# Future-Power-Networks/MAPDN

Hardware: AMD Instinct MI355X
Metric: env-steps/sec (whole node), case141 batch=4096, at 1/2/4/8 MI355X (higher is better)
Workload: dtype f64

## Files before the change

### mapdn_amd/csrc/critic.hip

```cpp
#include <hip/hip_runtime.h>
#include <stdint.h>

#include <algorithm>
#include <cstdlib>

#include "../../include/mapdn.h"
#include "rowtile.hpp"

namespace mapdn {

template <bool BC>
__device__ __forceinline__ void load_row(const HeadArgs& p, long row, int g, f4 (&xa)[4]) {
  if (BC) {
    const unsigned q = (unsigned)row / (unsigned)p.n, i = (unsigned)row - q * (unsigned)p.n;
    const float* pb = p.x + (size_t)q * 64 + 4 * g;
    const float* pn = p.per_n + (size_t)i * 64 + 4 * g;
#pragma unroll
    for (int c = 0; c < 4; ++c) xa[c] = *(const f4*)(pb + 16 * c) + *(const f4*)(pn + 16 * c);
  } else {
    const float* px = p.x + (size_t)row * 64 + 4 * g;
#pragma unroll
    for (int c = 0; c < 4; ++c) xa[c] = *(const f4*)(px + 16 * c);
  }
}

template <bool BC>
__global__ void __launch_bounds__(256)
k_head_fwd(HeadArgs p, float* __restrict__ v, long rows) {
  const int lane = threadIdx.x & 63, wave = threadIdx.x >> 6, g = lane >> 4, j = lane & 15;
  f4 wop[4][4], gam[4], bet[4], b2v[4], w3v[4];
#pragma unroll
  for (int nt = 0; nt < 4; ++nt) {
#pragma unroll
    for (int c = 0; c < 4; ++c) wop[nt][c] = *(const f4*)(p.w2 + (size_t)(16 * nt + j) * 64 + 16 * c + 4 * g);
    gam[nt] = *(const f4*)(p.gamma + 16 * nt + 4 * g); bet[nt] = *(const f4*)(p.beta + 16 * nt + 4 * g);
    b2v[nt] = *(const f4*)(p.b2 + 16 * nt + 4 * g); w3v[nt] = *(const f4*)(p.w3 + 16 * nt + 4 * g);
  }
  const float b3 = p.b3[0];
  const long n_tiles = (rows + 15) >> 4;
  for (long T = (long)blockIdx.x * 4 + wave; T < n_tiles; T += (long)gridDim.x * 4) {
    const long row = T * 16 + j;
    f4 xa[4];
    load_row<BC>(p, row < rows ? row : rows - 1, g, xa);
    ln_stats(xa, p.eps);
#pragma unroll
    for (int c = 0; c < 4; ++c) {
      const f4 y = xa[c] * gam[c] + bet[c];
      xa[c] = f4{relu_nan(y.x), relu_nan(y.y), relu_nan(y.z), relu_nan(y.w)};
    }
    f4 acc[4] = {f4{0, 0, 0, 0}, f4{0, 0, 0, 0}, f4{0, 0, 0, 0}, f4{0, 0, 0, 0}};
#pragma unroll
    for (int c = 0; c < 4; ++c)
#pragma unroll
      for (int q = 0; q < 4; ++q)
#pragma unroll
        for (int nt = 0; nt < 4; ++nt) acc[nt] = __builtin_amdgcn_mfma_f32_16x16x4f32(wop[nt][c][q], xa[c][q], acc[nt], 0, 0, 0);
    float dot = 0.0f;
#pragma unroll
    for (int nt = 0; nt < 4; ++nt)
#pragma unroll
      for (int r = 0; r < 4; ++r) dot = fmaf(relu_nan(acc[nt][r] + b2v[nt][r]), w3v[nt][r], dot);
    dot = sum_g(dot);
    if (g == 0 && row < rows) v[row] = dot + b3;
  }
}

template <bool BC, int MODE, int NT>
__global__ void __launch_bounds__(NT)
k_head_bwd(HeadArgs p, const float* __restrict__ dv, float* __restrict__ dx, const float* __restrict__ dot_w, float* __restrict__ dact,
           float* __restrict__ partial, int pstride, long rows, const float* __restrict__ wrow, const float* __restrict__ scale) {
  constexpr bool PG = MODE == 0 || MODE == 3;
  constexpr int NW = NT / 64, TILES = NT == 512 ? 1 : 2;
  constexpr bool SLIM = NT == 512;
  extern __shared__ float sm[];
  f4* sW = (f4*)sm;
  f4* sWT = sW + 1024;
  float* sP = (float*)(sWT + 1024);
  float* stage = sP + 256 + (size_t)(threadIdx.x >> 6) * TILES * 16 * HS;
  float* accn = sP + 256 + (size_t)NW * TILES * 16 * HS + (size_t)(threadIdx.x >> 6) * p.n * 64;
  const int tid = threadIdx.x, lane = tid & 63, wave = tid >> 6, g = lane >> 4, j = lane & 15;
  if (tid < 64) { sP[tid] = p.gamma[tid]; sP[64 + tid] = p.beta[tid]; sP[128 + tid] = p.b2[tid]; sP[192 + tid] = p.w3[tid]; }
  for (int i = tid; i < 1024; i += NT) {
    const int l = i & 63, c = (i >> 6) & 3, nt = i >> 8, lj = l & 15, lg = l >> 4;
    sW[i] = *(const f4*)(p.w2 + (size_t)(16 * nt + lj) * 64 + 16 * c + 4 * lg);
    f4 t;
#pragma unroll
    for (int q = 0; q < 4; ++q) t[q] = p.w2[(size_t)(16 * c + 4 * lg + q) * 64 + 16 * nt + lj];
    sWT[i] = t;
  }
  if (BC && MODE != 2) for (int i = lane; i < p.n * 64; i += 64) accn[i] = 0.0f;
  f4 gam_[4], bet_[4], b2v_[4], w3v_[4];
#pragma unroll
  for (int nt = 0; nt < 4; ++nt) {
    gam_[nt] = *(const f4*)(p.gamma + 16 * nt + 4 * g); bet_[nt] = *(const f4*)(p.beta + 16 * nt + 4 * g);
    b2v_[nt] = *(const f4*)(p.b2 + 16 * nt + 4 * g); w3v_[nt] = *(const f4*)(p.w3 + 16 * nt + 4 * g);
  }
  __syncthreads();
  auto GAM = [&](int c) -> f4 { return SLIM ? *(const f4*)(sP + 16 * c + 4 * g) : gam_[c]; };
  auto BET = [&](int c) -> f4 { return SLIM ? *(const f4*)(sP + 64 + 16 * c + 4 * g) : bet_[c]; };
  auto B2V = [&](int c) -> f4 { return SLIM ? *(const f4*)(sP + 128 + 16 * c + 4 * g) : b2v_[c]; };
  auto W3V = [&](int c) -> f4 { return SLIM ? *(const f4*)(sP + 192 + 16 * c + 4 * g) : w3v_[c]; };

  const long W = (long)gridDim.x * NW, w = (long)blockIdx.x * NW + wave;
  long r0, r1;
  if (BC) { const long G = rows / p.n; r0 = (G * w / W) * p.n; r1 = (G * (w + 1) / W) * p.n; }
  else { const long Tn = (rows + 15) >> 4; r0 = (Tn * w / W) * 16; r1 = (Tn * (w + 1) / W) * 16; if (r1 > rows) r1 = rows; }

  f4 accW[4][4];
  f4 ag[4], ab[4], aw3[4], ab2[4];
  float ab3 = 0.0f, carry = 0.0f;
  float aloss = 0.0f;
  const float b3 = MODE == 3 ? p.b3[0] : 0.0f, lscale = MODE == 3 ? scale[0] : 0.0f;
#pragma unroll
  for (int a = 0; a < 4; ++a) {
#pragma unroll
    for (int b = 0; b < 4; ++b) accW[a][b] = f4{0, 0, 0, 0};
    ag[a] = ab[a] = aw3[a] = ab2[a] = f4{0, 0, 0, 0};
  }

  f4 xnext[4];
  float dvnext = 0.0f;
  if (!SLIM && r0 < r1) {
    const long row = r0 + j;
    load_row<BC>(p, row < r1 ? row : r1 - 1, g, xnext);
    dvnext = row < r1 ? dv[row] : 0.0f;
  }
  for (long row0 = r0; row0 < r1; row0 += 16) {
    const long row = row0 + j;
    const bool valid = row < r1;
    f4 xh[4];
    float dvcur;
    if (SLIM) {
      load_row<BC>(p, valid ? row : r1 - 1, g, xh);
      dvcur = valid ? dv[row] : 0.0f;
    } else {
#pragma unroll
      for (int c = 0; c < 4; ++c) xh[c] = xnext[c];
      dvcur = dvnext;
      if (row0 + 16 < r1) {
        const long rn = row + 16;
        load_row<BC>(p, rn < r1 ? rn : r1 - 1, g, xnext);
        dvnext = rn < r1 ? dv[rn] : 0.0f;
      }
    }
    const float rs = ln_stats(xh, p.eps);
    f4 xn[4];
#pragma unroll
    for (int c = 0; c < 4; ++c) {
      const f4 y = xh[c] * GAM(c) + BET(c);
      xn[c] = f4{relu_nan(y.x), relu_nan(y.y), relu_nan(y.z), relu_nan(y.w)};
    }
    f4 acc[4] = {f4{0, 0, 0, 0}, f4{0, 0, 0, 0}, f4{0, 0, 0, 0}, f4{0, 0, 0, 0}};
#pragma unroll
    for (int c = 0; c < 4; ++c) {
      f4 wv[4];
#pragma unroll
      for (int nt = 0; nt < 4; ++nt) wv[nt] = sW[(nt * 4 + c) * 64 + lane];
#pragma unroll
      for (int q = 0; q < 4; ++q)
#pragma unroll
        for (int nt = 0; nt < 4; ++nt) acc[nt] = __builtin_amdgcn_mfma_f32_16x16x4f32(wv[nt][q], xn[c][q], acc[nt], 0, 0, 0);
    }
    float dvr = dvcur;
    if (MODE == 3) {
      float dot = 0.0f;
#pragma unroll
      for (int nt = 0; nt < 4; ++nt) {
        const f4 bb = B2V(nt), ww = W3V(nt);
#pragma unroll
        for (int r = 0; r < 4; ++r) dot = fmaf(relu_nan(acc[nt][r] + bb[r]), ww[r], dot);
      }
      const float err = dvcur - (sum_g(dot) + b3);
      float wgt = lscale;
      if (wrow) { const unsigned rc = (unsigned)(valid ? row : r1 - 1); wgt *= wrow[BC ? rc / (unsigned)p.n : rc]; }
      dvr = valid ? -2.0f * wgt * err : 0.0f;
      if (valid && g == 0) aloss = fmaf(wgt * err, err, aloss);
    }
#pragma unroll
    for (int nt = 0; nt < 4; ++nt) {
      const f4 bb = B2V(nt), ww = W3V(nt);
#pragma unroll
      for (int r = 0; r < 4; ++r) {
        const float pre = acc[nt][r] + bb[r];
        const bool pos = pre > 0.0f;
        const float dp = pos ? dvr * ww[r] : 0.0f;
        if (PG) { aw3[nt][r] = fmaf(pos ? pre : 0.0f, dvr, aw3[nt][r]); ab2[nt][r] += dp; }
        acc[nt][r] = dp;
      }
    }
    if (PG && g == 0) ab3 += dvr;
    f4 dxn[4] = {f4{0, 0, 0, 0}, f4{0, 0, 0, 0}, f4{0, 0, 0, 0}, f4{0, 0, 0, 0}};
#pragma unroll
    for (int c = 0; c < 4; ++c) {
      f4 wv[4];
#pragma unroll
      for (int nt = 0; nt < 4; ++nt) wv[nt] = sWT[(nt * 4 + c) * 64 + lane];
#pragma unroll
      for (int q = 0; q < 4; ++q)
#pragma unroll
        for (int nt = 0; nt < 4; ++nt) dxn[nt] = __builtin_amdgcn_mfma_f32_16x16x4f32(wv[nt][q], acc[c][q], dxn[nt], 0, 0, 0);
    }
    if (PG) {
      float* s0 = stage; float* s1 = SLIM ? stage : stage + 16 * HS;
#pragma unroll
      for (int c = 0; c < 4; ++c) *(f4*)(s0 + j * HS + 16 * c + 4 * g) = acc[c];
      if (!SLIM) {
#pragma unroll
        for (int c = 0; c < 4; ++c) *(f4*)(s1 + j * HS + 16 * c + 4 * g) = xn[c];
      }
      __builtin_amdgcn_fence(__ATOMIC_RELEASE, "wavefront");
      __builtin_amdgcn_wave_barrier();
      __builtin_amdgcn_fence(__ATOMIC_ACQUIRE, "wavefront");
      float dCs[4][4];
      if (SLIM) {
#pragma unroll
        for (int s = 0; s < 4; ++s)
#pragma unroll
          for (int nt = 0; nt < 4; ++nt) dCs[s][nt] = s0[(4 * g + s) * HS + 16 * nt + j];
        __builtin_amdgcn_fence(__ATOMIC_RELEASE, "wavefront");
        __builtin_amdgcn_wave_barrier();
#pragma unroll
        for (int c = 0; c < 4; ++c) *(f4*)(s1 + j * HS + 16 * c + 4 * g) = xn[c];
        __builtin_amdgcn_fence(__ATOMIC_RELEASE, "wavefront");
        __builtin_amdgcn_wave_barrier();
        __builtin_amdgcn_fence(__ATOMIC_ACQUIRE, "wavefront");
      }
#pragma unroll
      for (int s = 0; s < 4; ++s) {
        float dC[4], xC[4];
#pragma unroll
        for (int nt = 0; nt < 4; ++nt) { dC[nt] = SLIM ? dCs[s][nt] : s0[(4 * g + s) * HS + 16 * nt + j]; xC[nt] = s1[(4 * g + s) * HS + 16 * nt + j]; }
#pragma unroll
        for (int a = 0; a < 4; ++a)
#pragma unroll
          for (int b = 0; b < 4; ++b) accW[a][b] = __builtin_amdgcn_mfma_f32_16x16x4f32(dC[a], xC[b], accW[a][b], 0, 0, 0);
      }
    }
    float s1a = 0.0f, s2a = 0.0f;
#pragma unroll
    for (int c = 0; c < 4; ++c) {
      f4 d;
#pragma unroll
      for (int q = 0; q < 4; ++q) d[q] = xn[c][q] > 0.0f ? dxn[c][q] : 0.0f;
      if (PG) { ag[c] += d * xh[c]; ab[c] += d; }
      const f4 a = d * GAM(c);
      s1a += hsum(a); s2a += hsum(a * xh[c]);
      dxn[c] = a;
    }
    const float m1 = sum_g(s1a) * (1.0f / 64.0f), m2 = sum_g(s2a) * (1.0f / 64.0f);
#pragma unroll
    for (int c = 0; c < 4; ++c) dxn[c] = (dxn[c] - m1 - xh[c] * m2) * rs;
    if (MODE == 2) {
      const unsigned i = BC ? (unsigned)((valid ? row : r1 - 1) - r0) % (unsigned)p.n : 0u;
      const float* pw = dot_w + (size_t)i * 64 + 4 * g;
      float d = 0.0f;
#pragma unroll
      for (int c = 0; c < 4; ++c) d += hsum(dxn[c] * *(const f4*)(pw + 16 * c));
      d = sum_g(d);
      if (g == 0 && valid) dact[row] = d;
    } else if (!BC) {
      if (valid) {
        float* px = dx + (size_t)row * 64 + 4 * g;
#pragma unroll
        for (int c = 0; c < 4; ++c) *(f4*)(px + 16 * c) = dxn[c];
      }
    } else {
      float* s0 = stage;
      __builtin_amdgcn_fence(__ATOMIC_RELEASE, "wavefront");
      __builtin_amdgcn_wave_barrier();
#pragma unroll
      for (int c = 0; c < 4; ++c) *(f4*)(s0 + j * HS + 16 * c + 4 * g) = dxn[c];
      __builtin_amdgcn_fence(__ATOMIC_RELEASE, "wavefront");
      __builtin_amdgcn_wave_barrier();
      __builtin_amdgcn_fence(__ATOMIC_ACQUIRE, "wavefront");
      const int cnt = (int)(r1 - row0 < 16 ? r1 - row0 : 16);
      const unsigned rel = (unsigned)(row0 - r0);
      unsigned grp = rel / (unsigned)p.n, i = rel - grp * (unsigned)p.n;
      float* pbase = dx + ((size_t)(r0 / p.n) + grp) * 64 + lane;
      if (p.n >= 16) {
        unsigned i2 = i;
        constexpr int H = SLIM ? 4 : 16;
#pragma unroll
        for (int h0 = 0; h0 < 16; h0 += H) {
          float val[H], cur[H];
#pragma unroll
          for (int rr = 0; rr < H; ++rr) {
            unsigned ii = i + h0 + rr; if (ii >= (unsigned)p.n) ii -= p.n;
            val[rr] = h0 + rr < cnt ? s0[(h0 + rr) * HS + lane] : 0.0f;
            cur[rr] = accn[ii * 64 + lane];
          }
#pragma unroll
          for (int rr = 0; rr < H; ++rr) {
            unsigned ii = i + h0 + rr; if (ii >= (unsigned)p.n) ii -= p.n;
            accn[ii * 64 + lane] = cur[rr] + val[rr];
          }
#pragma unroll
          for (int rr = 0; rr < H; ++rr)
            if (h0 + rr < cnt) {
              carry += val[rr];
              if (++i2 == (unsigned)p.n) { *pbase = carry; carry = 0.0f; i2 = 0; pbase += 64; }
            }
        }
      } else {
        for (int rr = 0; rr < cnt; ++rr) {
          const float val = s0[rr * HS + lane];
          carry += val;
          accn[i * 64 + lane] += val;
          if (++i == (unsigned)p.n) { *pbase = carry; carry = 0.0f; i = 0; pbase += 64; }
        }
      }
      __builtin_amdgcn_fence(__ATOMIC_RELEASE, "wavefront");
      __builtin_amdgcn_wave_barrier();
    }
  }

  if (MODE != 2) {
    float* pp = partial + (size_t)blockIdx.x * pstride;
    if (BC) {
      __syncthreads();
      const float* a0 = sP + 256 + (size_t)NW * TILES * 16 * HS;
      for (int i = tid; i < p.n * 64; i += NT) {
        float t = a0[i];
#pragma unroll
        for (int ww = 1; ww < NW; ++ww) t += a0[(size_t)ww * p.n * 64 + i];
        pp[HP + i] = t;
      }
    }
    if (PG) {
      __syncthreads();
      float* red = sm + (size_t)wave * HP;
#pragma unroll
      for (int a = 0; a < 4; ++a)
#pragma unroll
        for (int b = 0; b < 4; ++b)
#pragma unroll
          for (int r = 0; r < 4; ++r) red[(16 * a + 4 * g + r) * 64 + 16 * b + j] = accW[a][b][r];
#pragma unroll
      for (int c = 0; c < 4; ++c)
#pragma unroll
        for (int q = 0; q < 4; ++q) {
          const float tg = sum_j(ag[c][q]), tb = sum_j(ab[c][q]), t2 = sum_j(ab2[c][q]), t3 = sum_j(aw3[c][q]);
          if (j == 0) {
            const int col = 16 * c + 4 * g + q;
            red[4096 + col] = tg; red[4160 + col] = tb; red[4224 + col] = t2; red[4288 + col] = t3;
          }
        }
      const float t = sum_j(ab3), tl = sum_j(aloss);
      if (lane == 0) { red[4352] = t; red[4353] = tl; }
      __syncthreads();
      for (int col = tid; col < HW; col += NT) {
        float v = sm[col];
#pragma unroll
        for (int ww = 1; ww < NW; ++ww) v += sm[(size_t)ww * HP + col];
        pp[col] = v;
      }
    }
  }
}

__global__ void __launch_bounds__(256) k_head_reduce(const float* __restrict__ partial, int nw, int pstride, int lo, int hi, int written,
                                                     float* __restrict__ out) {
  __shared__ float s_acc[4][64];
  const int c = threadIdx.x & 63, grp = threadIdx.x >> 6, col = lo + blockIdx.x * 64 + c;
  float acc = 0.0f;
  if (col < written) for (int i = grp; i < nw; i += 4) acc += partial[(size_t)i * pstride + col];
  s_acc[grp][c] = acc;
  __syncthreads();
  if (grp == 0 && col < hi) out[col] = (s_acc[0][c] + s_acc[1][c]) + (s_acc[2][c] + s_acc[3][c]);
}

}

static int head_cus() {
  int dev = 0, cus = 256;
  if (hipGetDevice(&dev) == hipSuccess) (void)hipDeviceGetAttribute(&cus, hipDeviceAttributeMultiprocessorCount, dev);
  return cus;
}
static int head_bwd_blocks(int64_t rows, int32_t n, bool bc, int nw, int cus = 0) {
  const int64_t units = bc ? rows / n : (rows + 15) / 16;
  return (int)std::max<int64_t>(1, std::min<int64_t>((units + nw - 1) / nw, cus ? cus : head_cus()));
}
static size_t head_bwd_lds(int threads, int32_t n, bool accn) {
  const int nw = threads / 64, tiles = threads == 512 ? 1 : 2;
  return (size_t)2 * 1024 * 16 + 256 * 4 + (size_t)nw * tiles * 16 * mapdn::HS * 4 + (accn ? (size_t)nw * n * 64 * 4 : 0);
}
static int head_bwd_threads(int64_t rows, int32_t n, bool bc, bool accn, int cus = 0) {
  const char* e = getenv("MAPDN_HEAD_BWD_THREADS");
  const bool fits = head_bwd_lds(512, n, accn) <= (size_t)160 * 1024;
  if (e && atoi(e) == 256) return 256;
  if (e && atoi(e) == 512 && fits) return 512;
  const int64_t units = bc ? rows / n : (rows + 15) / 16;
  return fits && units >= (int64_t)(cus ? cus : head_cus()) * 8 ? 512 : 256;
}
static bool head_args_ok(const float* x, const float* per_n, int32_t n, const float* gamma, const float* beta, const float* w2, const float* b2,
                         const float* w3, const float* b3, int64_t rows) {
  if (!x || !gamma || !beta || !w2 || !b2 || !w3 || !b3 || rows < 1 || rows > 0x7fffffff) return false;
  if (per_n && (n < 1 || n > 256 || rows % n)) return false;
  return true;
}

extern "C" int mapdn_critic_head_forward(const float* x, const float* per_n, int32_t n, const float* gamma, const float* beta, float eps,
                                         const float* w2, const float* b2, const float* w3, const float* b3, float* v, int64_t rows,
                                         void* stream) {
  using namespace mapdn;
  if (!head_args_ok(x, per_n, n, gamma, beta, w2, b2, w3, b3, rows) || !v) return MAPDN_E_INVALID;
  const HeadArgs a{x, per_n, per_n ? n : 1, gamma, beta, eps, w2, b2, w3, b3};
  const int64_t tiles = (rows + 15) / 16;
  const int blocks = (int)std::max<int64_t>(1, std::min<int64_t>((tiles + 3) / 4, (int64_t)head_cus() * 2));
  if (per_n) hipLaunchKernelGGL(k_head_fwd<true>, dim3(blocks), dim3(256), 0, (hipStream_t)stream, a, v, (long)rows);
  else hipLaunchKernelGGL(k_head_fwd<false>, dim3(blocks), dim3(256), 0, (hipStream_t)stream, a, v, (long)rows);
  return hipGetLastError() == hipSuccess ? MAPDN_OK : MAPDN_E_HIP;
}

extern "C" int64_t mapdn_critic_head_scratch_floats(int64_t rows, int32_t n, int32_t formed) {
  if (rows < 1 || (formed && (n < 1 || rows % n))) return 0;
  const int64_t blocks = std::max<int64_t>(head_bwd_blocks(rows, n, formed != 0, 4), head_bwd_blocks(rows, n, formed != 0, 8));
  return blocks * (mapdn::HP + (formed ? n * 64 : 0));
}

extern "C" int mapdn_critic_head_backward_geometry(int64_t rows, int32_t n, int32_t formed, int32_t mode, int32_t cus, int32_t* threads,
                                                   int32_t* blocks, int32_t* lds_bytes) {
  if (rows < 1 || rows > 0x7fffffff || mode < 0 || mode > 3 || cus < 0 || (formed && (n < 1 || n > 256 || rows % n))) return MAPDN_E_INVALID;
  const bool bc = formed != 0;
  if (!bc) n = 1;
  const int c = cus ? cus : head_cus();
  const int nt = head_bwd_threads(rows, n, bc, bc && mode != 2, c);
  size_t lds = head_bwd_lds(nt, n, bc && mode != 2);
  if (mode == 0 || mode == 3) lds = std::max(lds, (size_t)(nt / 64) * mapdn::HP * 4);
  if (lds > (size_t)160 * 1024) return MAPDN_E_INVALID;
  if (threads) *threads = nt;
  if (blocks) *blocks = head_bwd_blocks(rows, n, bc, nt / 64, c);
  if (lds_bytes) *lds_bytes = (int32_t)lds;
  return MAPDN_OK;
}

template <bool BC, int MODE, int NT>
static int head_bwd_launch_nt(const mapdn::HeadArgs& a, const float* dv, float* dx, const float* dot_w, float* dact, float* scratch, float* grads,
                              int64_t rows, hipStream_t st, const float* wrow, const float* scale) {
  using namespace mapdn;
  constexpr int NW = NT / 64;
  const int blocks = head_bwd_blocks(rows, a.n, BC, NW), nw = blocks;
  const int pstride = HP + (BC ? a.n * 64 : 0);
  size_t lds = head_bwd_lds(NT, a.n, BC && MODE != 2);
  if (MODE == 0 || MODE == 3) lds = std::max(lds, (size_t)NW * HP * 4);
  if (lds > (size_t)160 * 1024) return MAPDN_E_INVALID;
  const void* fn = (const void*)k_head_bwd<BC, MODE, NT>;
  if (hipFuncSetAttribute(fn, hipFuncAttributeMaxDynamicSharedMemorySize, 160 * 1024) != hipSuccess) return MAPDN_E_HIP;
  hipLaunchKernelGGL((k_head_bwd<BC, MODE, NT>), dim3(blocks), dim3(NT), lds, st, a, dv, dx, dot_w, dact, scratch, pstride, (long)rows, wrow, scale);
  if (MODE == 0 || MODE == 3) hipLaunchKernelGGL(k_head_reduce, dim3((HP + 63) / 64), dim3(256), 0, st, scratch, nw, pstride, 0, HP, HW, grads);
  if (BC && MODE != 2) hipLaunchKernelGGL(k_head_reduce, dim3(a.n), dim3(256), 0, st, scratch, nw, pstride, HP, HP + a.n * 64, HP + a.n * 64, grads);
  return hipGetLastError() == hipSuccess ? MAPDN_OK : MAPDN_E_HIP;
}
template <bool BC, int MODE>
static int head_bwd_launch(const mapdn::HeadArgs& a, const float* dv, float* dx, const float* dot_w, float* dact, float* scratch, float* grads,
                           int64_t rows, hipStream_t st, const float* wrow = nullptr, const float* scale = nullptr) {
  if (head_bwd_threads(rows, a.n, BC, BC && MODE != 2) == 512)
    return head_bwd_launch_nt<BC, MODE, 512>(a, dv, dx, dot_w, dact, scratch, grads, rows, st, wrow, scale);
  return head_bwd_launch_nt<BC, MODE, 256>(a, dv, dx, dot_w, dact, scratch, grads, rows, st, wrow, scale);
}

extern "C" int mapdn_critic_head_backward(const float* dv, const float* x, const float* per_n, int32_t n, const float* gamma, const float* beta,
                                          float eps, const float* w2, const float* b2, const float* w3, const float* b3, float* dx, float* grads,
                                          float* scratch, int64_t rows, int32_t param_grads, void* stream) {
  using namespace mapdn;
  if (!head_args_ok(x, per_n, n, gamma, beta, w2, b2, w3, b3, rows) || !dv || !dx || ((param_grads || per_n) && (!grads || !scratch)))
    return MAPDN_E_INVALID;
  const HeadArgs a{x, per_n, per_n ? n : 1, gamma, beta, eps, w2, b2, w3, b3};
  hipStream_t st = (hipStream_t)stream;
  if (per_n) return param_grads ? head_bwd_launch<true, 0>(a, dv, dx, nullptr, nullptr, scratch, grads, rows, st)
                                : head_bwd_launch<true, 1>(a, dv, dx, nullptr, nullptr, scratch, grads, rows, st);
  return param_grads ? head_bwd_launch<false, 0>(a, dv, dx, nullptr, nullptr, scratch, grads, rows, st)
                     : head_bwd_launch<false, 1>(a, dv, dx, nullptr, nullptr, scratch, grads, rows, st);
}

extern "C" int mapdn_critic_head_backward_dot(const float* dv, const float* x, const float* per_n, int32_t n, const float* gamma,
                                              const float* beta, float eps, const float* w2, const float* b2, const float* w3, const float* b3,
                                              const float* dot_w, float* dact, int64_t rows, void* stream) {
  using namespace mapdn;
  if (!head_args_ok(x, per_n, n, gamma, beta, w2, b2, w3, b3, rows) || !dv || !dot_w || !dact) return MAPDN_E_INVALID;
  const HeadArgs a{x, per_n, per_n ? n : 1, gamma, beta, eps, w2, b2, w3, b3};
  hipStream_t st = (hipStream_t)stream;
  return per_n ? head_bwd_launch<true, 2>(a, dv, nullptr, dot_w, dact, nullptr, nullptr, rows, st)
               : head_bwd_launch<false, 2>(a, dv, nullptr, dot_w, dact, nullptr, nullptr, rows, st);
}

extern "C" int mapdn_critic_head_mse(const float* ret, const float* wrow, const float* scale, const float* x, const float* per_n, int32_t n,
                                     const float* gamma, const float* beta, float eps, const float* w2, const float* b2, const float* w3,
                                     const float* b3, float* dx, float* grads, float* scratch, int64_t rows, void* stream) {
  using namespace mapdn;
  if (!head_args_ok(x, per_n, n, gamma, beta, w2, b2, w3, b3, rows) || !ret || !scale || !dx || !grads || !scratch) return MAPDN_E_INVALID;
  const HeadArgs a{x, per_n, per_n ? n : 1, gamma, beta, eps, w2, b2, w3, b3};
  hipStream_t st = (hipStream_t)stream;
  return per_n ? head_bwd_launch<true, 3>(a, ret, dx, nullptr, nullptr, scratch, grads, rows, st, wrow, scale)
               : head_bwd_launch<false, 3>(a, ret, dx, nullptr, nullptr, scratch, grads, rows, st, wrow, scale);
}

#include "critic_twin.hip"
#include "critic_cf.hip"
#include "critic_attn.hip"
```

Baseline: 39.98 million.

## Restructure critic backward row fetch with incremental indexing and vectorized staging

Replaces per-row integer division and modulo for broadcast group indexing with incrementally advanced counters, and folds row-weight and per-n loads into a unified prefetch lambda. LDS staging of activations and gradients now uses f4 vector reads with a transposed layout, and the xn store is moved earlier to overlap with the MFMA work. The weight-gradient reduction layout changes to match the new layout. It also swaps the relu helper and uses readfirstlane for the wave index. These changes aim to cut scalar address arithmetic and scalar LDS traffic, at the risk of subtle indexing or layout mismatches.

```diff
diff --git a/mapdn_amd/csrc/critic.hip b/mapdn_amd/csrc/critic.hip
--- a/mapdn_amd/csrc/critic.hip
+++ b/mapdn_amd/csrc/critic.hip
@@ -23,6 +23,18 @@
     for (int c = 0; c < 4; ++c) xa[c] = *(const f4*)(px + 16 * c);
   }
 }
+
+__device__ __forceinline__ float relu_keep(float o) { return !(o <= 0.0f) ? o : 0.0f; }
+
+__device__ __forceinline__ f4 ln_affine(f4 xh, f4 gam, f4 bet) {
+  return f4{fmaf(xh.x, gam.x, bet.x), fmaf(xh.y, gam.y, bet.y), fmaf(xh.z, gam.z, bet.z), fmaf(xh.w, gam.w, bet.w)};
+}
+
+__device__ __forceinline__ void stage_put(float* t, int j, int g, const f4 (&v)[4]) {
+#pragma unroll
+  for (int c = 0; c < 4; ++c) *(f4*)(t + j * HS + 16 * c + 4 * g) = v[c];
+}
+__device__ __forceinline__ f4 stage_get(const float* t, int j, int g, int s) { return *(const f4*)(t + (4 * g + s) * HS + 4 * j); }
 
 template <bool BC>
 __global__ void __launch_bounds__(256)
@@ -46,7 +58,7 @@
 #pragma unroll
     for (int c = 0; c < 4; ++c) {
       const f4 y = xa[c] * gam[c] + bet[c];
-      xa[c] = f4{relu_nan(y.x), relu_nan(y.y), relu_nan(y.z), relu_nan(y.w)};
+      xa[c] = f4{relu_keep(y.x), relu_keep(y.y), relu_keep(y.z), relu_keep(y.w)};
     }
     f4 acc[4] = {f4{0, 0, 0, 0}, f4{0, 0, 0, 0}, f4{0, 0, 0, 0}, f4{0, 0, 0, 0}};
 #pragma unroll
@@ -59,7 +71,7 @@
 #pragma unroll
     for (int nt = 0; nt < 4; ++nt)
 #pragma unroll
-      for (int r = 0; r < 4; ++r) dot = fmaf(relu_nan(acc[nt][r] + b2v[nt][r]), w3v[nt][r], dot);
+      for (int r = 0; r < 4; ++r) dot = fmaf(relu_keep(acc[nt][r] + b2v[nt][r]), w3v[nt][r], dot);
     dot = sum_g(dot);
     if (g == 0 && row < rows) v[row] = dot + b3;
   }
@@ -76,9 +88,9 @@
   f4* sW = (f4*)sm;
   f4* sWT = sW + 1024;
   float* sP = (float*)(sWT + 1024);
-  float* stage = sP + 256 + (size_t)(threadIdx.x >> 6) * TILES * 16 * HS;
-  float* accn = sP + 256 + (size_t)NW * TILES * 16 * HS + (size_t)(threadIdx.x >> 6) * p.n * 64;
-  const int tid = threadIdx.x, lane = tid & 63, wave = tid >> 6, g = lane >> 4, j = lane & 15;
+  const int tid = threadIdx.x, lane = tid & 63, wave = __builtin_amdgcn_readfirstlane(tid >> 6), g = lane >> 4, j = lane & 15;
+  float* stage = sP + 256 + (size_t)wave * TILES * 16 * HS;
+  float* accn = sP + 256 + (size_t)NW * TILES * 16 * HS + (size_t)wave * p.n * 64;
   if (tid < 64) { sP[tid] = p.gamma[tid]; sP[64 + tid] = p.beta[tid]; sP[128 + tid] = p.b2[tid]; sP[192 + tid] = p.w3[tid]; }
   for (int i = tid; i < 1024; i += NT) {
     const int l = i & 63, c = (i >> 6) & 3, nt = i >> 8, lj = l & 15, lg = l >> 4;
@@ -118,37 +130,61 @@
     ag[a] = ab[a] = aw3[a] = ab2[a] = f4{0, 0, 0, 0};
   }
 
-  f4 xnext[4];
-  float dvnext = 0.0f;
-  if (!SLIM && r0 < r1) {
-    const long row = r0 + j;
-    load_row<BC>(p, row < r1 ? row : r1 - 1, g, xnext);
-    dvnext = row < r1 ? dv[row] : 0.0f;
-  }
+  const unsigned un = (unsigned)p.n, dq = 16u / un, di = 16u % un;
+  const unsigned g0 = BC ? (unsigned)(r0 / p.n) : 0u, qlast = BC ? (unsigned)((r1 - 1) / p.n) : 0u;
+  unsigned fq = BC ? g0 + (unsigned)j / un : 0u, fi = BC ? (unsigned)j % un : 0u, fg = g0, fti = 0, tg = g0, ti = 0;
+
+  f4 nxa[4], nxb[4];
+  float ndv = 0.0f, nwr = 1.0f;
+  unsigned ni = 0;
+  auto fetch = [&](long row0f) {
+    const bool ok = row0f + j < r1;
+    const char* xb;
+    unsigned rel;
+    if (BC) {
+      rel = (ok ? fq : qlast) - fg;
+      ni = ok ? fi : un - 1;
+      xb = (const char*)(p.x + (size_t)fg * 64);
+      const unsigned poff = ni * 256u + 16u * g;
+#pragma unroll
+      for (int c = 0; c < 4; ++c) nxb[c] = *(const f4*)((const char*)p.per_n + poff + 64 * c);
+      if (MODE == 3 && wrow) nwr = *(const float*)((const char*)(wrow + fg) + 4u * rel);
+      fi += di; fq += dq;
+      if (fi >= un) { fi -= un; ++fq; }
+      fti += di; fg += dq;
+      if (fti >= un) { fti -= un; ++fg; }
+    } else {
+      rel = ok ? (unsigned)j : (unsigned)(r1 - 1 - row0f);
+      xb = (const char*)(p.x + (size_t)row0f * 64);
+      if (MODE == 3 && wrow) nwr = *(const float*)((const char*)(wrow + row0f) + 4u * rel);
+    }
+    const unsigned off = rel * 256u + 16u * g;
+#pragma unroll
+    for (int c = 0; c < 4; ++c) nxa[c] = *(const f4*)(xb + off + 64 * c);
+    ndv = ok ? *(const float*)((const char*)(dv + row0f) + 4u * j) : 0.0f;
+  };
+  if (!SLIM && r0 < r1) fetch(r0);
   for (long row0 = r0; row0 < r1; row0 += 16) {
-    const long row = row0 + j;
-    const bool valid = row < r1;
+    const bool valid = row0 + j < r1;
+    if (SLIM) fetch(row0);
     f4 xh[4];
-    float dvcur;
-    if (SLIM) {
-      load_row<BC>(p, valid ? row : r1 - 1, g, xh);
-      dvcur = valid ? dv[row] : 0.0f;
-    } else {
-#pragma unroll
-      for (int c = 0; c < 4; ++c) xh[c] = xnext[c];
-      dvcur = dvnext;
-      if (row0 + 16 < r1) {
-        const long rn = row + 16;
-        load_row<BC>(p, rn < r1 ? rn : r1 - 1, g, xnext);
-        dvnext = rn < r1 ? dv[rn] : 0.0f;
-      }
-    }
+#pragma unroll
+    for (int c = 0; c < 4; ++c) xh[c] = BC ? nxa[c] + nxb[c] : nxa[c];
+    const float dvcur = ndv, wcur = nwr;
+    const unsigned icur = ni;
+    if (!SLIM && row0 + 16 < r1) fetch(row0 + 16);
     const float rs = ln_stats(xh, p.eps);
     f4 xn[4];
 #pragma unroll
     for (int c = 0; c < 4; ++c) {
-      const f4 y = xh[c] * GAM(c) + BET(c);
-      xn[c] = f4{relu_nan(y.x), relu_nan(y.y), relu_nan(y.z), relu_nan(y.w)};
+      const f4 y = ln_affine(xh[c], GAM(c), BET(c));
+      xn[c] = f4{relu_keep(y.x), relu_keep(y.y), relu_keep(y.z), relu_keep(y.w)};
+    }
+    float* s0 = stage; float* s1 = SLIM ? stage : stage + 16 * HS;
+    if (PG && !SLIM) {
+      __builtin_amdgcn_fence(__ATOMIC_RELEASE, "wavefront");
+      __builtin_amdgcn_wave_barrier();
+      stage_put(s1, j, g, xn);
     }
     f4 acc[4] = {f4{0, 0, 0, 0}, f4{0, 0, 0, 0}, f4{0, 0, 0, 0}, f4{0, 0, 0, 0}};
 #pragma unroll
@@ -168,11 +204,11 @@
       for (int nt = 0; nt < 4; ++nt) {
         const f4 bb = B2V(nt), ww = W3V(nt);
 #pragma unroll
-        for (int r = 0; r < 4; ++r) dot = fmaf(relu_nan(acc[nt][r] + bb[r]), ww[r], dot);
+        for (int r = 0; r < 4; ++r) dot = fmaf(relu_keep(acc[nt][r] + bb[r]), ww[r], dot);
       }
       const float err = dvcur - (sum_g(dot) + b3);
       float wgt = lscale;
-      if (wrow) { const unsigned rc = (unsigned)(valid ? row : r1 - 1); wgt *= wrow[BC ? rc / (unsigned)p.n : rc]; }
+      if (wrow) wgt *= wcur;
       dvr = valid ? -2.0f * wgt * err : 0.0f;
       if (valid && g == 0) aloss = fmaf(wgt * err, err, aloss);
     }
@@ -184,11 +220,18 @@
         const float pre = acc[nt][r] + bb[r];
         const bool pos = pre > 0.0f;
         const float dp = pos ? dvr * ww[r] : 0.0f;
-        if (PG) { aw3[nt][r] = fmaf(pos ? pre : 0.0f, dvr, aw3[nt][r]); ab2[nt][r] += dp; }
+        if (PG) { aw3[nt][r] = fmaf(MODE == 3 ? relu_keep(pre) : (pos ? pre : 0.0f), dvr, aw3[nt][r]); ab2[nt][r] += dp; }
         acc[nt][r] = dp;
       }
     }
     if (PG && g == 0) ab3 += dvr;
+    if (PG) {
+      if (SLIM) {
+        __builtin_amdgcn_fence(__ATOMIC_RELEASE, "wavefront");
+        __builtin_amdgcn_wave_barrier();
+      }
+      stage_put(s0, j, g, acc);
+    }
     f4 dxn[4] = {f4{0, 0, 0, 0}, f4{0, 0, 0, 0}, f4{0, 0, 0, 0}, f4{0, 0, 0, 0}};
 #pragma unroll
     for (int c = 0; c < 4; ++c) {
@@ -201,35 +244,23 @@
         for (int nt = 0; nt < 4; ++nt) dxn[nt] = __builtin_amdgcn_mfma_f32_16x16x4f32(wv[nt][q], acc[c][q], dxn[nt], 0, 0, 0);
     }
     if (PG) {
-      float* s0 = stage; float* s1 = SLIM ? stage : stage + 16 * HS;
-#pragma unroll
-      for (int c = 0; c < 4; ++c) *(f4*)(s0 + j * HS + 16 * c + 4 * g) = acc[c];
-      if (!SLIM) {
-#pragma unroll
-        for (int c = 0; c < 4; ++c) *(f4*)(s1 + j * HS + 16 * c + 4 * g) = xn[c];
-      }
       __builtin_amdgcn_fence(__ATOMIC_RELEASE, "wavefront");
       __builtin_amdgcn_wave_barrier();
       __builtin_amdgcn_fence(__ATOMIC_ACQUIRE, "wavefront");
-      float dCs[4][4];
+      f4 dCs[4];
       if (SLIM) {
 #pragma unroll
-        for (int s = 0; s < 4; ++s)
-#pragma unroll
-          for (int nt = 0; nt < 4; ++nt) dCs[s][nt] = s0[(4 * g + s) * HS + 16 * nt + j];
+        for (int s = 0; s < 4; ++s) dCs[s] = stage_get(s0, j, g, s);
         __builtin_amdgcn_fence(__ATOMIC_RELEASE, "wavefront");
         __builtin_amdgcn_wave_barrier();
-#pragma unroll
-        for (int c = 0; c < 4; ++c) *(f4*)(s1 + j * HS + 16 * c + 4 * g) = xn[c];
+        stage_put(s1, j, g, xn);
         __builtin_amdgcn_fence(__ATOMIC_RELEASE, "wavefront");
         __builtin_amdgcn_wave_barrier();
         __builtin_amdgcn_fence(__ATOMIC_ACQUIRE, "wavefront");
       }
 #pragma unroll
       for (int s = 0; s < 4; ++s) {
-        float dC[4], xC[4];
-#pragma unroll
-        for (int nt = 0; nt < 4; ++nt) { dC[nt] = SLIM ? dCs[s][nt] : s0[(4 * g + s) * HS + 16 * nt + j]; xC[nt] = s1[(4 * g + s) * HS + 16 * nt + j]; }
+        const f4 dC = SLIM ? dCs[s] : stage_get(s0, j, g, s), xC = stage_get(s1, j, g, s);
 #pragma unroll
         for (int a = 0; a < 4; ++a)
 #pragma unroll
@@ -251,21 +282,19 @@
 #pragma unroll
     for (int c = 0; c < 4; ++c) dxn[c] = (dxn[c] - m1 - xh[c] * m2) * rs;
     if (MODE == 2) {
-      const unsigned i = BC ? (unsigned)((valid ? row : r1 - 1) - r0) % (unsigned)p.n : 0u;
-      const float* pw = dot_w + (size_t)i * 64 + 4 * g;
+      const char* pw = (const char*)dot_w + ((BC ? icur : 0u) * 256u + 16u * g);
       float d = 0.0f;
 #pragma unroll
-      for (int c = 0; c < 4; ++c) d += hsum(dxn[c] * *(const f4*)(pw + 16 * c));
+      for (int c = 0; c < 4; ++c) d += hsum(dxn[c] * *(const f4*)(pw + 64 * c));
       d = sum_g(d);
-      if (g == 0 && valid) dact[row] = d;
+      if (g == 0 && valid) *(float*)((char*)(dact + row0) + 4u * j) = d;
     } else if (!BC) {
       if (valid) {
-        float* px = dx + (size_t)row * 64 + 4 * g;
-#pragma unroll
-        for (int c = 0; c < 4; ++c) *(f4*)(px + 16 * c) = dxn[c];
+        char* px = (char*)(dx + (size_t)row0 * 64) + (j * 256u + 16u * g);
+#pragma unroll
+        for (int c = 0; c < 4; ++c) *(f4*)(px + 64 * c) = dxn[c];
       }
     } else {
-      float* s0 = stage;
       __builtin_amdgcn_fence(__ATOMIC_RELEASE, "wavefront");
       __builtin_amdgcn_wave_barrier();
 #pragma unroll
@@ -274,9 +303,8 @@
       __builtin_amdgcn_wave_barrier();
       __builtin_amdgcn_fence(__ATOMIC_ACQUIRE, "wavefront");
       const int cnt = (int)(r1 - row0 < 16 ? r1 - row0 : 16);
-      const unsigned rel = (unsigned)(row0 - r0);
-      unsigned grp = rel / (unsigned)p.n, i = rel - grp * (unsigned)p.n;
-      float* pbase = dx + ((size_t)(r0 / p.n) + grp) * 64 + lane;
+      unsigned i = ti;
+      float* pbase = dx + (size_t)tg * 64 + lane;
       if (p.n >= 16) {
         unsigned i2 = i;
         constexpr int H = SLIM ? 4 : 16;
@@ -285,20 +313,20 @@
           float val[H], cur[H];
 #pragma unroll
           for (int rr = 0; rr < H; ++rr) {
-            unsigned ii = i + h0 + rr; if (ii >= (unsigned)p.n) ii -= p.n;
+            unsigned ii = i + h0 + rr; if (ii >= un) ii -= un;
             val[rr] = h0 + rr < cnt ? s0[(h0 + rr) * HS + lane] : 0.0f;
             cur[rr] = accn[ii * 64 + lane];
           }
 #pragma unroll
           for (int rr = 0; rr < H; ++rr) {
-            unsigned ii = i + h0 + rr; if (ii >= (unsigned)p.n) ii -= p.n;
+            unsigned ii = i + h0 + rr; if (ii >= un) ii -= un;
             accn[ii * 64 + lane] = cur[rr] + val[rr];
           }
 #pragma unroll
           for (int rr = 0; rr < H; ++rr)
             if (h0 + rr < cnt) {
               carry += val[rr];
-              if (++i2 == (unsigned)p.n) { *pbase = carry; carry = 0.0f; i2 = 0; pbase += 64; }
+              if (++i2 == un) { *pbase = carry; carry = 0.0f; i2 = 0; pbase += 64; }
             }
         }
       } else {
@@ -306,9 +334,11 @@
           const float val = s0[rr * HS + lane];
           carry += val;
           accn[i * 64 + lane] += val;
-          if (++i == (unsigned)p.n) { *pbase = carry; carry = 0.0f; i = 0; pbase += 64; }
+          if (++i == un) { *pbase = carry; carry = 0.0f; i = 0; pbase += 64; }
         }
       }
+      ti += di; tg += dq;
+      if (ti >= un) { ti -= un; ++tg; }
       __builtin_amdgcn_fence(__ATOMIC_RELEASE, "wavefront");
       __builtin_amdgcn_wave_barrier();
     }
@@ -334,7 +364,7 @@
 #pragma unroll
         for (int b = 0; b < 4; ++b)
 #pragma unroll
-          for (int r = 0; r < 4; ++r) red[(16 * a + 4 * g + r) * 64 + 16 * b + j] = accW[a][b][r];
+          for (int r = 0; r < 4; ++r) red[(4 * (4 * g + r) + a) * 64 + 4 * j + b] = accW[a][b][r];
 #pragma unroll
       for (int c = 0; c < 4; ++c)
 #pragma unroll
```

After: 39.53 million. 1.1% lower.
